# edwindn/rl-agent-for-qubit-array-tuning

Hardware: AMD Instinct MI355X
Metric: env steps/sec (batched 8-dot 64x64 CSD solves) (higher is better)
Workload: dtype f64; 1 GPU; 8-dot array, 4096 parallel envs per GPU, 64x64 CSD, deterministic physics (latching/noise off), 50-step episodes, staggered phases: 820 episode resets (new device + first observation) inside the timed region, synthetic CNN outputs; n_dots=8, envs_per_gpu=4096, resolution=64

## Files before the change

__graft_entry__.py:

```python
import os
import subprocess
import sys

ROOT = os.path.dirname(os.path.abspath(__file__))
PKG = os.path.join(ROOT, "rl-agent-for-qubit-array-tuning_amd")
for _p in (PKG, os.path.join(ROOT, "oracle"), os.path.join(ROOT, "tests")):
    if _p not in sys.path:
        sys.path.insert(0, _p)


def build() -> None:
    csrc = os.path.join(PKG, "csrc")
    subprocess.check_call(["make", "-C", csrc, "libqdsim.so"])
    subprocess.check_call(["make", "-C", os.path.join(ROOT, "tests", "hosttest"), "libqdsim_hosttest.so"])
    subprocess.check_call(["make", "-C", os.path.join(ROOT, "tests", "hosttest_wave"), "libqdsim_hosttest_wave.so"])
    subprocess.check_call(["make", "-C", os.path.join(ROOT, "oracle"), "libqdoracle.so"])
    import qadapt_hip
    from qadapt_hip import _lib
    L = _lib.lib()
    missing = [n for n in _lib.EXPORTS if not hasattr(L, n)]
    if missing:
        raise RuntimeError(f"libqdsim.so lacks symbols: {missing}")


def smoke() -> None:
    import numpy as np
    import torch
    import qd_oracle as O
    import helpers as H
    from qadapt_hip.vec_env import VecQuantumDeviceEnv, SyntheticCapacitanceModel

    assert torch.cuda.is_available(), "smoke() needs the MI355X"
    N, R, B, seed = 4, 16, 2, 2024
    env = VecQuantumDeviceEnv(B, num_dots=N, resolution=R, seed=seed, validate=True,
                              capacitance_model=SyntheticCapacitanceModel(3))
    rng = np.random.default_rng(0)
    C = N - 1
    v0 = rng.normal(0, 0.1, (B, C, 3)).astype(np.float32); l0 = rng.uniform(-6, -2, (B, C, 3)).astype(np.float32)
    obs = env.reset(cnn_outputs=(torch.as_tensor(v0).cuda(), torch.as_tensor(l0).cuda()))
    act = rng.uniform(-1, 1, (B, 2 * N - 1)).astype(np.float32)
    v1 = rng.normal(0, 0.1, (B, C, 3)).astype(np.float32); l1 = rng.uniform(-6, -2, (B, C, 3)).astype(np.float32)
    obs, rew, term, trunc = env.step(torch.as_tensor(act).cuda(),
                                     cnn_outputs=(torch.as_tensor(v1).cuda(), torch.as_tensor(l1).cuda()))
    img = obs["image"].cpu().numpy()
    raw, _ = env.raw()
    for e in range(B):
        oe = O.OracleEnv(N, R)
        oe.reset(O.sample_episode(np.random.default_rng(seed + e), N), v0[e], l0[e])
        oobs, (gr, br), _, _ = oe.step(act[e, :N], act[e, N:], v1[e], l1[e])
        r = rew[e].cpu().numpy()
        assert np.allclose(r[:N], gr, rtol=1e-9) and np.allclose(r[N:], br, rtol=1e-9), "reward mismatch"
        H.image_parity(oe, img[e], raw[e])
    env.close()
    print("smoke ok: 4-dot 16x16 batched step matches the oracle")


if __name__ == "__main__":
    build()
    if len(sys.argv) > 1 and sys.argv[1] == "smoke":
        smoke()
```

include/qdsim.h:

```cpp
#ifndef QDSIM_H
#define QDSIM_H

#include <stdint.h>

#ifdef __cplusplus
extern "C" {
#endif

#define QD_OK 0
#define QD_ERR_ARG 1
#define QD_ERR_HIP 2
#define QD_ERR_STATE 3
#define QD_ERR_NOMEM 4

#define QD_FLAG_VALIDATE 1
#define QD_FLAG_PIXEL_SEARCH 2
#define QD_FLAG_RETIRED_TILE_FUSED 4

#define QD_NOISE_SENSOR 1
#define QD_NOISE_RADIAL 2
#define QD_NOISE_LATCH 4

typedef struct qd_handle qd_handle;

typedef struct qd_config {
    int32_t struct_size;
    int32_t n_dot;
    int32_t resolution;
    int32_t batch;
    int32_t max_steps;
    int32_t env_chunk;
    int32_t flags;
    int32_t noise_flags;
    double gate_ramp_start;
    double gate_quadratic_start;
    double barrier_ramp_start;
    double kalman_prior_mean;
    double kalman_prior_variance;
    double kalman_prior_mean_nnn;
    double kalman_variance_threshold;
    double kalman_process_noise;
    uint64_t rng_seed;
    int64_t env_id_offset;
    int32_t use_deltas;
    int32_t sparse_reward;
    int32_t gate_curve_type;
    int32_t update_method;
    int32_t cnn_outputs;
    int32_t num_charge_states;
    double delta_max;
    double gate_curve_exponent;
    double plunger_radius;
    double outer_plunger_radius;
    double outer_plunger_reward_max;
    double barrier_radius;
} qd_config;

#define QD_ALL_CHARGE_STATES(m) (-(m))

#define QD_CURVE_CONSTANT 0
#define QD_CURVE_POLYNOMIAL 1
#define QD_CURVE_EXPONENTIAL 2
#define QD_CURVE_LINEAR 3
#define QD_UPDATE_KALMAN 0
#define QD_UPDATE_DIRECT 1

int qd_param_block_doubles(int n_dot);
int qd_state_block_doubles(int n_dot);
int qd_layout_query(int n_dot, int32_t* out31);
// ... 60 lines not shown
```

rl-agent-for-qubit-array-tuning_amd/csrc/qd_api.hip:

```cpp
#include <hip/hip_runtime.h>
#include <stdio.h>
#include <stdlib.h>
#include <string.h>
#include <new>

#include "qdsim.h"
#include "qd_kernels.h"
#include "qd_fullspace.h"
#include "qd_probe.h"

#define QD_MAX_LANES 4
struct QdLane {
    QdPixelRec* recs; unsigned char* slabs; unsigned* gtiles;
    unsigned char* wide;
    hipStream_t run, side, side2;
    hipEvent_t ev_fork, ev_join, ev_join2, ev_done;
};

struct qd_handle {
    qd_config cfg;
    QdLane lanes[QD_MAX_LANES]; int nlanes;
    hipEvent_t ev_start;
    int device;
    QdLayout L;
    int N, R, B, C, P;
    int chunk;
    double *params, *state, *zraw, *plohi, *occ, *eig;
    int* steps;
    QdPixelRec* recs;
    size_t recs_envs;
    float *gimg, *pimg, *bimg, *volt;
    unsigned long long* tel; int tel_words;
    unsigned long long* tstats;
    int tile_search;
    int kept, kc;
    int full_m;
    QdFullTab* ftab;
    int full_spl;
    QdWide wide;
    int ppb;
    unsigned char* slabs;
    unsigned* gtiles;
    int gs_chunk;
    size_t gs_batches;
    int cus;
    double* stage[2]; size_t stage_cap;
    hipEvent_t stage_ev[2]; int stage_turn;
    bool stage_busy[2];
    hipStream_t side, side2;
    hipEvent_t ev_fork, ev_join, ev_join2;
    unsigned long long obs_serial;
    double *pparams, *pstate, *pz, *pplohi;
    double *cz, *cplohi; size_t cz_cap, cplohi_cap;
    QdSelState* sel;
    char err[512];
};

static void qd_use_lane(qd_handle* h, int k) {
    const QdLane& ln = h->lanes[k];
    h->recs = ln.recs; h->slabs = ln.slabs; h->gtiles = ln.gtiles; h->wide.buf = ln.wide;
    h->side = ln.side; h->side2 = ln.side2; h->ev_fork = ln.ev_fork; h->ev_join = ln.ev_join; h->ev_join2 = ln.ev_join2;
}

static int qd_fail(qd_handle* h, int code, const char* what, hipError_t e = hipSuccess) {
    if (h) {
        if (e != hipSuccess) snprintf(h->err, sizeof(h->err), "%s: %s", what, hipGetErrorString(e));
        else snprintf(h->err, sizeof(h->err), "%s", what);
    }
    return code;
}
#define QD_HIP(call)                                                              \
    do { hipError_t e_ = (call); if (e_ != hipSuccess) return qd_fail(h, QD_ERR_HIP, #call, e_); } while (0)

struct QdDeviceGuard {
    int prev; bool switched; hipError_t err;
    explicit QdDeviceGuard(int dev) : prev(-1), switched(false), err(hipSuccess) {
        err = hipGetDevice(&prev);
        if (err == hipSuccess && prev != dev) { err = hipSetDevice(dev); switched = (err == hipSuccess); }
    }
    ~QdDeviceGuard() { if (switched) (void)hipSetDevice(prev); }
};
#define QD_ON_DEVICE(h)                                                           \
    QdDeviceGuard guard_((h)->device);                                            \
    if (guard_.err != hipSuccess) return qd_fail((h), QD_ERR_HIP, "hipSetDevice", guard_.err)

struct QdEventPair {
    hipEvent_t a, b; bool ok;
// ... 16 lines not shown
        case 8: { constexpr int NN = 8; __VA_ARGS__; } break;                            \
        default: return qd_fail(h, QD_ERR_ARG, "n_dot must be in 2..8");          \
    }

#define QD_DISPATCH_KC(KC_, ...)                                                  \
    switch (KC_) {                                                                \
        case 8: { constexpr int KK = 8; __VA_ARGS__; } break;                            \
        case 16: { constexpr int KK = 16; __VA_ARGS__; } break;                          \
        case 32: { constexpr int KK = 32; __VA_ARGS__; } break;                          \
        default: return qd_fail(h, QD_ERR_ARG, "kept-set size must be 8, 16 or 32");     \
    }

extern "C" int qd_param_block_doubles(int n) { return (n < 2 || n > QD_MAXN) ? -1 : qd_layout(n).size; }
extern "C" int qd_state_block_doubles(int n) { return (n < 2 || n > QD_MAXN) ? -1 : qd_layout(n).s_size; }
extern "C" int qd_layout_query(int n, int32_t* out) {
    if (n < 2 || n > QD_MAXN || !out) return QD_ERR_ARG;
    QdLayout L = qd_layout(n);
    memcpy(out, &L, sizeof(L));
    return QD_OK;
}

static void qd_kalman_priors(const qd_config& cfg, int N, double* km, double* kv) {
    for (int i = 0; i < N * N; ++i) { km[i] = 0.0; kv[i] = 0.0; }
    for (int i = 0; i < N - 1; ++i) {
        km[i * N + i + 1] = km[(i + 1) * N + i] = cfg.kalman_prior_mean;
        kv[i * N + i + 1] = kv[(i + 1) * N + i] = cfg.kalman_prior_variance;
    }
    if (cfg.cnn_outputs != 2)
        for (int i = 0; i < N - 2; ++i) {
            km[i * N + i + 2] = km[(i + 2) * N + i] = cfg.kalman_prior_mean_nnn;
            kv[i * N + i + 2] = kv[(i + 2) * N + i] = cfg.kalman_prior_variance;
        }
}

extern "C" const char* qd_last_error(const qd_handle* h) { return h ? h->err : "null handle"; }

extern "C" int qd_create(const qd_config* cfg, int device, qd_handle** out) {
    if (!cfg || !out || cfg->struct_size != (int32_t)sizeof(qd_config)) return QD_ERR_ARG;
    if (cfg->n_dot < 2 || cfg->n_dot > QD_MAXN || cfg->resolution < 2 || cfg->batch < 1) return QD_ERR_ARG;
    if (cfg->cnn_outputs != 2 && cfg->cnn_outputs != 3) return QD_ERR_ARG;
    if (cfg->gate_curve_type < 0 || cfg->gate_curve_type > 3 || cfg->update_method < 0 || cfg->update_method > 1) return QD_ERR_ARG;
    if (cfg->flags & QD_FLAG_RETIRED_TILE_FUSED) return QD_ERR_ARG;
    if (cfg->num_charge_states > QD_K) return QD_ERR_ARG;
    if (cfg->num_charge_states < 0 && !qd_full_supported(cfg->n_dot, -cfg->num_charge_states)) return QD_ERR_ARG;
    qd_handle* h = new (std::nothrow) qd_handle();
    if (!h) return QD_ERR_NOMEM;
    memset(h, 0, sizeof(*h));
    h->cfg = *cfg; h->device = device;
    h->N = cfg->n_dot; h->R = cfg->resolution; h->B = cfg->batch;
    h->C = h->N - 1; h->P = h->R * h->R; h->L = qd_layout(h->N);
    h->kept = cfg->num_charge_states > 0 ? cfg->num_charge_states : QD_K;
    h->kc = h->kept <= 8 ? 8 : (h->kept <= 16 ? 16 : 32);
    h->full_m = cfg->num_charge_states < 0 ? -cfg->num_charge_states : 0;
    *out = h;
    QD_ON_DEVICE(h);
    const bool val = (cfg->flags & QD_FLAG_VALIDATE) != 0;
    QdFullTab ftab;
    h->ppb = QD_GS_PPB;
    if (h->full_m) {
        qd_full_build(h->N, h->full_m, ftab);
        h->ppb = qd_full_ppb(ftab, val);
        if (h->ppb < 1) return qd_fail(h, QD_ERR_ARG, "the full charge-state space of this shape does not fit a slab");
        h->full_spl = qd_full_spl(ftab.M);
        if (qd_full_wide(ftab.maxsec)) h->wide.capw = (unsigned)((h->ppb * qd_full_wide_tasks(ftab) + 1) & ~1);
        QD_HIP(hipMalloc(&h->ftab, sizeof(QdFullTab)));
        QD_HIP(hipMemcpy(h->ftab, &ftab, sizeof(QdFullTab), hipMemcpyHostToDevice));
    }
    const size_t per_env_rec = (size_t)h->C * h->P * sizeof(QdPixelRec);
    const size_t batches_per_env = (size_t)h->C * ((h->P + h->ppb - 1) / h->ppb);
    const size_t per_env_slab = batches_per_env * (qd_gs_slab_bytes(val) + 4 * (qd_gs_tile_off(QD_GS_NBIN, 1)) + qd_wide_bytes(h->wide.capw));
    size_t budget = (size_t)64 << 30, free_b = 0, total_b = 0;
    if (const char* gib = getenv("QDSIM_SCRATCH_GIB")) { const long g = atol(gib); if (g > 0) budget = (size_t)g << 30; }
    if (hipMemGetInfo(&free_b, &total_b) == hipSuccess && free_b / 3 < budget) budget = free_b / 3;
    int chunk = cfg->env_chunk, gs_chunk;
    h->nlanes = 1;
    if (val) {
        chunk = h->B;
        size_t g = budget / per_env_slab;
        gs_chunk = (int)(g < 1 ? 1 : (g > (size_t)h->B ? (size_t)h->B : g));
        if (cfg->env_chunk > 0 && cfg->env_chunk < gs_chunk) gs_chunk = cfg->env_chunk;
    } else {
        h->nlanes = 2;
        if (const char* ls = getenv("QDSIM_LANES")) { const int l = atoi(ls); if (l >= 1 && l <= QD_MAX_LANES) h->nlanes = l; }
        if (chunk <= 0) {
            size_t g = budget / h->nlanes / (per_env_rec + per_env_slab);
            chunk = (int)(g < 1 ? 1 : g);
        }
        if (const char* cs = getenv("QDSIM_CHUNK")) { const int c = atoi(cs); if (c >= 1) chunk = c; }
        if (chunk >= h->B) {
            const int half = (h->B + 1) / 2;
            if (h->nlanes >= 2 && cfg->env_chunk <= 0 && (size_t)half * batches_per_env >= 2048) chunk = half;
            else { chunk = h->B; h->nlanes = 1; }
        }
        gs_chunk = chunk;
    }
    if ((size_t)gs_chunk * batches_per_env > ((size_t)1 << 20) - 1) {
        gs_chunk = (int)((((size_t)1 << 20) - 1) / batches_per_env);
        if (gs_chunk < 1) return qd_fail(h, QD_ERR_ARG, "resolution too large for the tile descriptors");
        if (!val && chunk > gs_chunk) chunk = gs_chunk;
    }
    h->chunk = chunk; h->recs_envs = (size_t)chunk;
    h->gs_chunk = gs_chunk; h->gs_batches = (size_t)gs_chunk * batches_per_env;
    {
        hipDeviceProp_t prop;
        QD_HIP(hipGetDeviceProperties(&prop, device));
        h->cus = prop.multiProcessorCount;
// ... 166 lines not shown
                   c.plunger_radius, c.outer_plunger_radius, c.outer_plunger_reward_max, c.barrier_radius};
    const int blk = 64, grd = (h->B + blk - 1) / blk;
    QD_DISPATCH_N(h->N, qd_k_actions<NN><<<dim3(grd), dim3(blk), 0, s>>>(h->B, h->params,
                                            h->state, h->steps, actions, rewards, truncated, rc));
    QD_HIP(hipGetLastError());
    return QD_OK;
}

static int qd_cand_blocks(int R) {
    const int tiles = ((R + 7) / 8) * ((R + 7) / 8), per_block = QD_CAND_BLOCK / 64;
    return (tiles + per_block - 1) / per_block;
}

static QdNoiseCfg qd_noise_cfg(const qd_handle* h) {
    QdNoiseCfg nz;
    nz.flags = h->cfg.noise_flags;
    nz.seed = (uint32_t)(h->cfg.rng_seed ^ (h->cfg.rng_seed >> 32));
    nz.env_off = (uint32_t)h->cfg.env_id_offset;
    nz.ser_lo = (uint32_t)h->obs_serial; nz.ser_hi = (uint32_t)(h->obs_serial >> 32);
    nz.tel = h->tel; nz.tel_words = h->tel_words;
    return nz;
}

template <int BIN>
static hipError_t qd_launch_solve(qd_handle* h, hipStream_t s) {
    static int per_cu[2] = {0, 0};
    const int v = h->eig ? 1 : 0;
    if (!per_cu[v]) {
        int n = 0;
        const hipError_t e = v ? hipOccupancyMaxActiveBlocksPerMultiprocessor(&n, qd_k_gs_solve<BIN, true>, 256, 0)
                               : hipOccupancyMaxActiveBlocksPerMultiprocessor(&n, qd_k_gs_solve<BIN, false>, 256, 0);
        if (e != hipSuccess) return e;
        per_cu[v] = n < 1 ? 1 : n;
    }
    const dim3 grid((unsigned)(h->cus * per_cu[v]));
    unsigned* tilelist = h->gtiles + 16;
    if (h->eig) qd_k_gs_solve<BIN, true><<<grid, dim3(256), 0, s>>>(h->slabs, h->gtiles, tilelist, h->gs_batches, h->tstats);
    else        qd_k_gs_solve<BIN, false><<<grid, dim3(256), 0, s>>>(h->slabs, h->gtiles, tilelist, h->gs_batches, nullptr);
    return hipGetLastError();
}

static int qd_launch_ground(qd_handle* h, const int32_t* env_ids, int base, int cnt, hipStream_t s, int stages = 7 ) {
    const int nb = (h->P + h->ppb - 1) / h->ppb;
    unsigned* tilelist = h->gtiles + 16;
    const int rec0 = (h->cfg.flags & QD_FLAG_VALIDATE) ? base : 0;
    for (int off = 0; off < cnt; off += h->gs_chunk) {
        const int n = cnt - off < h->gs_chunk ? cnt - off : h->gs_chunk;
        const QdGsGeom g{n, h->C, h->P, nb};
        const unsigned batches = (unsigned)((size_t)n * h->C * nb);
        if (stages & 1) {
        QD_HIP(hipMemsetAsync(h->gtiles, 0, sizeof(unsigned) * 16, s));
#define QD_LAUNCH_STRUCTURE(VAL_, WPB_)                                                                                          \
        QD_DISPATCH_N(h->N, qd_k_gs_structure<NN, VAL_, WPB_><<<dim3(batches), dim3(64 * WPB_), 0, s>>>(env_ids, base + off, rec0 + off, g, h->R, \
                      h->params, h->recs, h->state, h->cfg.noise_flags, h->slabs, h->gtiles, tilelist, h->gs_batches, h->kept))
        const bool small = batches < (unsigned)h->cus;
        if (h->full_m) {
#define QD_LAUNCH_FULL(VAL_, SPL_, WIDE_)                                                                                         \
            QD_DISPATCH_N(h->N, qd_k_full_structure<NN, VAL_, SPL_, WIDE_><<<dim3(batches), dim3(64 * QdFullWpb<SPL_>::v), 0, s>>>(env_ids,    \
                          base + off, rec0 + off, g, h->ppb, h->R, h->params, h->state, h->cfg.noise_flags, h->ftab, h->recs, h->slabs,   \
                          h->gtiles, tilelist, h->gs_batches, h->wide))
#define QD_LAUNCH_FULL_V(VAL_)                                                                                                    \
            do {                                                                                                                  \
                if (!h->wide.capw && h->full_spl == 2) { QD_LAUNCH_FULL(VAL_, 2, false); }                                        \
                else if (h->full_spl == 2) { QD_LAUNCH_FULL(VAL_, 2, true); }                                                     \
                else if (h->full_spl == 4) { QD_LAUNCH_FULL(VAL_, 4, true); }                                                     \
                else { QD_LAUNCH_FULL(VAL_, 8, true); }                                                                           \
            } while (0)
            if (h->eig) QD_LAUNCH_FULL_V(true); else QD_LAUNCH_FULL_V(false);
#undef QD_LAUNCH_FULL_V
#undef QD_LAUNCH_FULL
        } else if (h->eig) { if (small) { QD_LAUNCH_STRUCTURE(true, 16); } else { QD_LAUNCH_STRUCTURE(true, 4); } }
        else        { if (small) { QD_LAUNCH_STRUCTURE(false, 16); } else { QD_LAUNCH_STRUCTURE(false, 4); } }
#undef QD_LAUNCH_STRUCTURE
        QD_HIP(hipGetLastError());
        }
        if (stages & 2) {
        int max_bin = h->N == 2 ? qd_gs_bin(4) : (h->N == 3 ? qd_gs_bin(12) : QD_GS_NBIN - 1);
        if (h->full_m) {
            int M = 0, maxsec = 0;
            qd_full_sizes(h->N, h->full_m, M, maxsec);
            max_bin = qd_gs_bin(maxsec < QD_K ? maxsec : QD_K);
        } else if (h->kept < 2) max_bin = -1;
        else if (qd_gs_bin(h->kept) < max_bin) max_bin = qd_gs_bin(h->kept);
        const bool forked = max_bin >= 9;
        hipStream_t s9 = forked ? h->side : s, s48 = forked ? h->side2 : s;
        if (forked) {
            QD_HIP(hipEventRecord(h->ev_fork, s));
            QD_HIP(hipStreamWaitEvent(h->side, h->ev_fork, 0));
            QD_HIP(hipStreamWaitEvent(h->side2, h->ev_fork, 0));
        }
        if (h->wide.capw) {
            const size_t slots = (size_t)batches * h->wide.capw, full = (size_t)h->cus * 4;
            const dim3 wgrid((unsigned)(slots < full ? slots : full));
            if (h->eig) qd_k_full_solve_wide<true><<<wgrid, dim3(64), 0, s>>>(h->slabs, h->wide, batches, h->tstats);
            else        qd_k_full_solve_wide<false><<<wgrid, dim3(64), 0, s>>>(h->slabs, h->wide, batches, nullptr);
            QD_HIP(hipGetLastError());
        }
        if (max_bin >= 9) QD_HIP(qd_launch_solve<9>(h, s9));
        if (forked) QD_HIP(hipEventRecord(h->ev_join, h->side));
        if (max_bin >= 8) QD_HIP(qd_launch_solve<8>(h, s48));
        if (max_bin >= 7) QD_HIP(qd_launch_solve<7>(h, s48));
        if (max_bin >= 6) QD_HIP(qd_launch_solve<6>(h, s48));
        if (max_bin >= 5) QD_HIP(qd_launch_solve<5>(h, s48));
        if (max_bin >= 4) QD_HIP(qd_launch_solve<4>(h, s48));
        if (forked) QD_HIP(hipEventRecord(h->ev_join2, h->side2));
        if (max_bin >= 0) QD_HIP(qd_launch_solve<0>(h, s));
        if (max_bin >= 1) QD_HIP(qd_launch_solve<1>(h, s));
// ... 520 lines not shown
```

rl-agent-for-qubit-array-tuning_amd/csrc/qd_groundstate.h:

```cpp
#pragma once
#include "qd_pixel.h"
#include "qd_eig.h"

#if defined(__HIPCC__)

#ifndef QD_NBREG
#define QD_NBREG 6
#endif
#define QD_GS_BLOCK 256
#define QD_GS_PPB 256
#define QD_GS_NBIN 10
__host__ __device__ inline int qd_gs_bin(int s) { return s <= 8 ? s - 2 : (s <= 10 ? 7 : (s <= 12 ? 8 : 9)); }
__host__ __device__ inline int qd_gs_bin_min(int bin) { return bin <= 6 ? bin + 2 : (bin == 7 ? 9 : (bin == 8 ? 11 : 13)); }
#define QD_LINK_NONE 0xFFFFFFFFu
#define QD_LINK_SINGLE 0xFFFFFFFEu

typedef __attribute__((address_space(3))) double qd_lds_double;
typedef volatile qd_lds_double* qd_lds_vptr;
typedef const volatile qd_lds_double* qd_lds_cvptr;

template <int N>
struct QdWaveLds {
    static constexpr int NS = (2 * (N - 1) - QD_NBREG) > 1 ? (2 * (N - 1) - QD_NBREG) : 1;
    double coef[NS][64];
    unsigned char nidx[NS][64];
    double buf[64];
    double pv[2][16];
    short pfl[2][8];
};
struct QdBlockLds {
    unsigned pool_top;
    unsigned cnt[QD_GS_NBIN];
};

struct QdSlab {
    double* pool; unsigned* link; unsigned char* rank; unsigned* lists; double* aux; unsigned* cnt; double* lam;
};
__host__ __device__ inline int qd_gs_list_cap(int bin) { return QD_GS_PPB * (32 / qd_gs_bin_min(bin)); }
__host__ __device__ inline int qd_gs_list_off(int bin) { int o = 0; for (int b = 0; b < bin; ++b) o += qd_gs_list_cap(b); return o; }
__host__ __device__ inline int qd_gs_task_doubles(int s, bool validate) {
    const int ne = s * (s + 1) / 2;
    const int n = 2 + ne + (s > QD_EIG_REG ? 4 * s + (validate ? ne : 0) : 0);
    return (n + 1) & ~1;
}
__host__ __device__ inline size_t qd_gs_pool_doubles(bool validate) { return (size_t)QD_GS_PPB * (size_t)qd_gs_task_doubles(32, validate); }
__host__ __device__ inline size_t qd_gs_slab_bytes(bool validate) {
    size_t b = qd_gs_pool_doubles(validate) * 8;
    b += (size_t)QD_GS_PPB * 32 * 4;
    b += (size_t)qd_gs_list_off(QD_GS_NBIN) * 4;
    b += (size_t)QD_GS_PPB * 16;
    b += (size_t)QD_GS_PPB * 32;
    b += 64;
    b += (size_t)qd_gs_list_off(QD_GS_NBIN) * 8;
    return (b + 255) & ~(size_t)255;
}
__host__ __device__ inline QdSlab qd_gs_slab(unsigned char* base, bool validate) {
    QdSlab s;
    s.pool = (double*)base; base += qd_gs_pool_doubles(validate) * 8;
    s.link = (unsigned*)base; base += (size_t)QD_GS_PPB * 32 * 4;
    s.lists = (unsigned*)base; base += (size_t)qd_gs_list_off(QD_GS_NBIN) * 4;
    s.aux = (double*)base; base += (size_t)QD_GS_PPB * 16;
    s.rank = base; base += (size_t)QD_GS_PPB * 32;
    s.cnt = (unsigned*)base; base += 64;
    s.lam = (double*)base;
    return s;
}
__host__ __device__ inline size_t qd_gs_tile_cap(int bin, size_t batches) { return batches * (size_t)((qd_gs_list_cap(bin) + 63) / 64); }
__host__ __device__ inline size_t qd_gs_tile_off(int bin, size_t batches) { size_t o = 0; for (int b = 0; b < bin; ++b) o += qd_gs_tile_cap(b, batches); return o; }

__device__ __forceinline__ unsigned qd_half_ballot(bool p) {
    unsigned long long b = __ballot(p);
    return (unsigned)(b >> (threadIdx.x & 32));
}
__device__ __forceinline__ double qd_half_min(double v) {
#pragma unroll
    for (int o = 16; o > 0; o >>= 1) v = fmin(v, __shfl_xor(v, o, 32));
    return v;
}
__device__ __forceinline__ int qd_wave_max_int(int v) {
#pragma unroll
    for (int o = 32; o > 0; o >>= 1) v = max(v, __shfl_xor(v, o, 64));
    return __builtin_amdgcn_readfirstlane(v);
}

template <int N, bool VALIDATE>
__device__ __forceinline__ void qd_ground_structure(const QdPixelRec* __restrict__ rec, bool live, int ps, QdWaveLds<N>& W,
                                                    QdBlockLds& S, const QdSlab& sl, int kept) {
    const int lane = threadIdx.x & 63;
    const int m = lane & 31;
    const int hb = lane & 32;
    const unsigned lt = (1u << m) - 1u;
    qd_lds_vptr buf = (qd_lds_vptr)W.buf;

    const int hh = hb >> 5;
    if (m >= 9 && m < 9 + N - 1) W.pv[hh][m] = rec->tc[m - 9];
    if (m >= 16 && m < 16 + N) W.pfl[hh][m - 16] = (short)rec->fl[m - 16];
    __builtin_amdgcn_wave_barrier();
    const double* pvv = W.pv[hh];
    const bool inK = m < kept;
    const int nvalid = min(rec->nvalid, kept);
    const bool valid = m < nvalid;
    const unsigned code = valid ? (unsigned)rec->idx[m] : 0u;
    unsigned ecode = code;
    ecode = (ecode | (ecode << 8)) & 0x00FF00FFu;
    ecode = (ecode | (ecode << 4)) & 0x0F0F0F0Fu;
    ecode = (ecode | (ecode << 2)) & 0x33333333u;
    const double Fabs = inK ? rec->E[m] : INFINITY;
    const double fshift = qd_half_min(Fabs);
    const double F = Fabs - fshift;

    unsigned tcnz = 0;
#pragma unroll
    for (int d = 0; d < N - 1; ++d) tcnz |= (pvv[9 + d] != 0.0 ? 1u : 0u) << d;
    unsigned tcq = 0;
#pragma unroll
    for (int q = 0; q < N - 1; ++q) tcq |= ((tcnz >> (N - 2 - q)) & 1u) << (4 * q);
    unsigned nbrmask = 0;
#pragma unroll 4
    for (int j = 1; j <= 16; ++j) {
        const int pj = (m + j) & 31;
        const unsigned cj = __shfl(ecode, pj, 32);
        const unsigned Z = ((cj | 0x88888888u) - ecode) ^ 0x88888888u;
        const int tz = __builtin_ctz(Z | 0x80000000u);
        const unsigned Zs = Z >> tz;
        const unsigned hop = ((unsigned)(Zs == 0x1Fu) | (unsigned)(Zs == 0xF1u)) & (tcq >> tz) & 1u;
        nbrmask |= hop << pj;
        if (j < 16) {
            const int qj = (m - j) & 31;
            const unsigned back = (unsigned)__shfl((int)hop, qj, 32);
            nbrmask |= back << qj;
        }
    }
    nbrmask = (valid && live) ? (nbrmask & (nvalid >= 32 ? 0xFFFFFFFFu : ((1u << nvalid) - 1u))) : 0u;
#if defined(QD_ABLATE) && QD_ABLATE == 4
    nbrmask = 0;
#endif
    const int cnt = __popc(nbrmask);
    const int maxcnt = qd_wave_max_int(cnt);
    double radius = 0.0;
    double creg[QD_NBREG]; int jreg[QD_NBREG];
#pragma unroll
    for (int i = 0; i < QD_NBREG; ++i) { creg[i] = 0.0; jreg[i] = m; }
    {
        unsigned rem = nbrmask;
        for (int s = 0; s < maxcnt; ++s) {
            const bool has = rem != 0;
            const int j = has ? __builtin_ctz(rem) : m;
            rem &= rem - 1;
            const unsigned cj = __shfl(ecode, j, 32);
            double c = 0.0;
            if (has) {
                const int Y = (int)cj - (int)ecode;
                const unsigned ay = (unsigned)(Y < 0 ? -Y : Y);
                const int q = __builtin_ctz(ay) >> 2;
                const int d = N - 2 - q;
                const int nd = (int)W.pfl[hh][d] + (int)((ecode >> (4 * (q + 1))) & 3u) - 1;
                const int nd1 = (int)W.pfl[hh][d + 1] + (int)((ecode >> (4 * q)) & 3u) - 1;
                const double t = pvv[9 + d];
                const double prod = (Y < 0) ? (double)nd * ((double)nd1 + 1.0)
                                            : (double)nd1 * ((double)nd + 1.0);
                double sq_ = 0.0;
                if (prod > 0.0) sq_ = qd_sqrt1(prod);
                c = -t * sq_;
            }
            if (s < QD_NBREG) {
#pragma unroll
                for (int i = 0; i < QD_NBREG; ++i) if (i == s) { creg[i] = c; jreg[i] = j; }
            } else { W.coef[s - QD_NBREG][lane] = c; W.nidx[s - QD_NBREG][lane] = (unsigned char)j; }
            radius += fabs(c);
        }
    }

    unsigned seg = (1u << m) | nbrmask;
    for (int guard = 0; guard < 32; ++guard) {
        unsigned nw = seg, rem = nbrmask;
        for (int s = 0; s < maxcnt; ++s) {
            const bool has = rem != 0;
            const int j = has ? __builtin_ctz(rem) : m;
            rem &= rem - 1;
            nw |= __shfl(seg, j, 32);
        }
        const bool changed = nw != seg;
        seg = nw;
        if (!__any(changed)) break;
    }
    const int ssz = __popc(seg);
    const int r = __popc(seg & lt);
    const int smax = qd_wave_max_int(ssz);

    double comp_lower;
    {
        buf[lane] = F - radius;
        __builtin_amdgcn_wave_barrier();
        double acc = INFINITY;
        unsigned mm = seg;
        for (int it = 0; it < smax; ++it) {
            if (mm) { const int b = __builtin_ctz(mm); mm &= mm - 1; acc = fmin(acc, buf[hb + b]); }
        }
        __builtin_amdgcn_wave_barrier();
        comp_lower = acc;
    }
    const bool active = live && comp_lower <= 0.0;
#if defined(QD_ABLATE) && QD_ABLATE == 3
    const bool solve = false;
#else
    const bool solve = active && ssz > 1;
#endif

    unsigned base = 0, gi = 0;
    if (solve && r == 0) {
        base = atomicAdd(&S.pool_top, (unsigned)qd_gs_task_doubles(ssz, VALIDATE));
        const int bin = qd_gs_bin(ssz);
        gi = (unsigned)qd_gs_list_off(bin) + atomicAdd(&S.cnt[bin], 1u);
        sl.lists[gi] = base;
        if (ssz > 8) sl.pool[base + 1] = (double)ssz;
    }
    base = (unsigned)__shfl((int)base, __builtin_ctz(seg), 32);
    gi = (unsigned)__shfl((int)gi, __builtin_ctz(seg), 32);
    if (live) {
        sl.link[ps * 32 + m] = solve ? gi : (active ? QD_LINK_SINGLE : QD_LINK_NONE);
        sl.rank[ps * 32 + m] = (unsigned char)r;
        if (VALIDATE) {
            const double hn = -qd_half_min(inK ? -(fabs(Fabs) + radius) : INFINITY);
            if (m == 0) { sl.aux[ps] = hn; sl.aux[QD_GS_PPB + ps] = fshift; }
        }
    }
    {
        double* row = sl.pool + base + 2 + (r * (r + 1)) / 2;
        unsigned nrm = 0;
        for (int s = 0; s < maxcnt; ++s) {
            if (s < cnt && solve) {
                int j = jreg[0]; double c = creg[0];
                if (s >= QD_NBREG) { j = (int)W.nidx[s - QD_NBREG][lane]; c = W.coef[s - QD_NBREG][lane]; }
#pragma unroll
                for (int i = 1; i < QD_NBREG; ++i) if (i == s) { j = jreg[i]; c = creg[i]; }
                const int rj = __popc(seg & ((1u << j) - 1u));
                if (rj < r) { row[rj] = c; nrm |= 1u << rj; }
            }
        }
        for (int c = 0; c < smax - 1; ++c)
            if (solve && c < r && !((nrm >> c) & 1u)) row[c] = 0.0;
        if (solve) row[r] = F;
    }
}

template <int S, bool PADDED, bool VALIDATE>
__device__ __forceinline__ int qd_eig_task(double* rec, double& lam) {
    double resid, x[S];
    int its = 0;
    const int sz = PADDED ? (int)rec[1] : S;
    qd_eig_lowest<S, VALIDATE>(rec + 2, lam, x, resid, VALIDATE ? &its : nullptr, sz);
    if (VALIDATE) rec[1] = resid;
    if (sz == S) {
        double2* X2 = reinterpret_cast<double2*>(rec + 2);
#pragma unroll
// ... 102 lines not shown
```

rl-agent-for-qubit-array-tuning_amd/csrc/qd_kernels.h:

```cpp
#pragma once
#include "qd_groundstate.h"
#include "qd_rng.h"

#if defined(__HIPCC__)

struct QdRewardCfg {
    double gate_ramp_start, gate_quadratic_start, barrier_ramp_start;
    int max_steps;
    int use_deltas, sparse, curve;
    double delta_max, curve_exponent;
    double plunger_radius, outer_plunger_radius, outer_plunger_reward_max, barrier_radius;
};

__device__ __forceinline__ double qd_gate_reward(double dist, const QdRewardCfg& rc) {
    if (rc.sparse) {
        if (dist <= rc.plunger_radius) return 1.0;
        if (dist <= rc.outer_plunger_radius) {
            const double nd = (dist - rc.plunger_radius) / (rc.outer_plunger_radius - rc.plunger_radius);
            return rc.outer_plunger_reward_max * (1.0 - nd);
        }
        return 0.0;
    }
    double r;
    if (dist >= rc.gate_ramp_start) r = 0.0;
// ... 163 lines not shown
    if (nv < KC) {
        double dd[N];
#pragma unroll
        for (int i = 0; i < N; ++i) dd[i] = 0.0 - vd[i];
#pragma unroll 1
        for (int i = 0; i < N; ++i) {
            const double t = qd_dotN<N>(spar + L.cdd_inv + i * G, dd);
            double di = dd[0];
#pragma unroll
            for (int j = 1; j < N; ++j) di = (j == i) ? dd[j] : di;
            F0 = fma(di, t, F0);
        }
    }
#pragma unroll
    for (int m = 0; m < KC; ++m) rec->E[m] = (m < nv ? se[m * QD_CAND_BLOCK + threadIdx.x] : F0) * isa;
#pragma unroll
    for (int i = 0; i < N; ++i) rec->fl[i] = fl[i];
    rec->nvalid = nv;
}

struct QdGsGeom { int n_env, C, P, nb; };
__device__ __forceinline__ void qd_gs_locate(const QdGsGeom& g, int batch, int& slot, int& ch, int& p0) {
    slot = batch / (g.C * g.nb);
    const int rem = batch - slot * g.C * g.nb;
    ch = rem / g.nb; p0 = (rem - ch * g.nb) * QD_GS_PPB;
}

__device__ __forceinline__ void qd_gs_publish_tiles(const QdBlockLds& sB, const QdSlab& sl, int batch, unsigned* __restrict__ gtiles,
                                                    unsigned* __restrict__ tilelist, size_t batches_cap) {
    if (threadIdx.x < QD_GS_NBIN) {
        const int bin = threadIdx.x;
        const unsigned nt = sB.cnt[bin];
        sl.cnt[bin] = nt;
        const unsigned ntile = (nt + 63u) >> 6;
        if (ntile) {
            const unsigned start = atomicAdd(&gtiles[bin], ntile);
            unsigned* tl = tilelist + qd_gs_tile_off(bin, batches_cap) + start;
            for (unsigned t = 0; t < ntile; ++t) {
                const unsigned here = nt - t * 64u < 64u ? nt - t * 64u : 64u;
                tl[t] = ((unsigned)batch << 12) | (t << 6) | (here - 1u);
            }
        }
    }
}

#ifndef QD_GS_WAVES
#define QD_GS_WAVES 7
#endif
template <int N, bool VALIDATE, int WPB>
__global__ void __launch_bounds__(64 * WPB, WPB == 4 ? QD_GS_WAVES : 4)
qd_k_gs_structure(const int* __restrict__ env_ids, int env_base, int rec_slot0, QdGsGeom g, int R, const double* __restrict__ params,
                  const QdPixelRec* __restrict__ recs, const double* __restrict__ state, int noise_flags,
                  unsigned char* __restrict__ slabs, unsigned* __restrict__ gtiles, unsigned* __restrict__ tilelist, size_t batches_cap,
                  int kept) {
    const QdLayout L = qd_layout(N);
    __shared__ QdWaveLds<N> sW[WPB];
    __shared__ QdBlockLds sB;
    constexpr int PPW = QD_GS_PPB / WPB;
    const int batch = blockIdx.x;
    const QdSlab sl = qd_gs_slab(slabs + (size_t)batch * qd_gs_slab_bytes(VALIDATE), VALIDATE);
    const int wave = threadIdx.x >> 6, lane = threadIdx.x & 63;
    int slot, ch, p0;
    qd_gs_locate(g, batch, slot, ch, p0);
    const int e = env_ids ? env_ids[env_base + slot] : env_base + slot;
    const double* par = params + (size_t)e * L.size;
    const double* st = state + (size_t)e * L.s_size;
    if (qd_radial_replaced(par, st, L, ch, noise_flags)) {
        if (threadIdx.x < QD_GS_NBIN) sl.cnt[threadIdx.x] = 0;
        return;
    }
    const QdPixelRec* rbase = recs + ((size_t)(rec_slot0 + slot) * g.C + ch) * g.P;
    if (threadIdx.x <= QD_GS_NBIN) { if (threadIdx.x == 0) sB.pool_top = 0; else sB.cnt[threadIdx.x - 1] = 0; }
    __syncthreads();
    QdWaveLds<N>& W = sW[wave];
    for (int it = 0; it < PPW / 2; ++it) {
        const int ps = wave * PPW + it * 2 + (lane >> 5);
        if (p0 + wave * PPW + it * 2 >= g.P) break;
        const int p = p0 + ps;
        const int pc = p < g.P ? p : g.P - 1;
        qd_ground_structure<N, VALIDATE>(rbase + pc, p < g.P, ps, W, sB, sl, kept);
    }
    __syncthreads();
    qd_gs_publish_tiles(sB, sl, batch, gtiles, tilelist, batches_cap);
}

template <int BIN, bool VALIDATE>
__device__ __forceinline__ int qd_gs_solve_task(double* rec, double& lam) {
    if constexpr (BIN <= 6) return qd_eig_task<BIN + 2, false, VALIDATE>(rec, lam);
    else if constexpr (BIN == 7) return qd_eig_task<10, true, VALIDATE>(rec, lam);
    else if constexpr (BIN == 8) return qd_eig_task<12, true, VALIDATE>(rec, lam);
    else return qd_eig_task_mem<VALIDATE>(rec, lam);
}
template <int BIN> struct QdGsSolveWaves { static constexpr int v = BIN <= 1 ? 6 : (BIN == 2 ? 4 : (BIN == 3 ? 3 : (BIN <= 6 ? 2 : (BIN == 9 ? 4 : 1)))); };

template <int BIN, bool VALIDATE>
__global__ void __launch_bounds__(256, QdGsSolveWaves<BIN>::v)
qd_k_gs_solve(unsigned char* __restrict__ slabs, const unsigned* __restrict__ gtiles, const unsigned* __restrict__ tilelist,
              size_t batches_cap, unsigned long long* __restrict__ stats) {
    const int lane = threadIdx.x & 63;
    const unsigned ntile = gtiles[BIN];
    const unsigned* tl = tilelist + qd_gs_tile_off(BIN, batches_cap);
    const unsigned nwaves = gridDim.x * 4u;
    unsigned gt = blockIdx.x * 4u + (threadIdx.x >> 6);
    const size_t slab_bytes = qd_gs_slab_bytes(VALIDATE);
    auto offset_of = [&](unsigned d) -> unsigned {
        const QdSlab sl = qd_gs_slab(slabs + (size_t)(d >> 12) * slab_bytes, VALIDATE);
        return lane <= (int)(d & 63u) ? sl.lists[qd_gs_list_off(BIN) + (int)((d >> 6) & 63u) * 64 + lane] : 0u;
    };
    unsigned desc = gt < ntile ? tl[gt] : 0u;
    unsigned desc1 = gt + nwaves < ntile ? tl[gt + nwaves] : 0u;
    unsigned off = gt < ntile ? offset_of(desc) : 0u;
    for (; gt < ntile; gt += nwaves) {
        const unsigned desc2 = gt + 2u * nwaves < ntile ? tl[gt + 2u * nwaves] : 0u;
        const unsigned off1 = gt + nwaves < ntile ? offset_of(desc1) : 0u;
        const unsigned batch = desc >> 12;
        const int here = (int)(desc & 63u) + 1;
        const QdSlab sl = qd_gs_slab(slabs + (size_t)batch * slab_bytes, VALIDATE);
        int its = 0;
        if (lane < here) {
            double lam;
            its = qd_gs_solve_task<BIN, VALIDATE>(sl.pool + off, lam);
            sl.lam[qd_gs_list_off(BIN) + (int)((desc >> 6) & 63u) * 64 + lane] = lam;
        }
        desc = desc1; desc1 = desc2; off = off1;
        if (VALIDATE && stats) {
            int sum = its, mx = its;
#pragma unroll
            for (int o = 32; o > 0; o >>= 1) { sum += __shfl_xor(sum, o, 64); mx = max(mx, __shfl_xor(mx, o, 64)); }
            if (lane == 0) {
                atomicAdd(&stats[16], (unsigned long long)here); atomicAdd(&stats[17], (unsigned long long)sum);
                atomicAdd(&stats[18], 1ull); atomicAdd(&stats[19], (unsigned long long)mx);
                atomicAdd(&stats[20 + BIN], (unsigned long long)here);
            }
// ... 579 lines not shown
```

rl-agent-for-qubit-array-tuning_amd/qadapt_hip/_lib.py:

```python
from __future__ import annotations

import ctypes
import os
import subprocess

_HERE = os.path.dirname(os.path.abspath(__file__))
CSRC = os.path.join(os.path.dirname(_HERE), "csrc")
LIB_PATH = os.environ.get("QDSIM_LIB", os.path.join(CSRC, "libqdsim.so"))

QD_FLAG_VALIDATE = 1
QD_FLAG_PIXEL_SEARCH = 2
QD_NOISE_SENSOR = 1
QD_NOISE_RADIAL = 2
QD_NOISE_LATCH = 4
QD_MAP_GLOBAL, QD_MAP_PER_SCAN = 0, 1
QD_ERR_ARG, QD_ERR_HIP, QD_ERR_STATE = 1, 2, 3

EXPORTS = [
    "qd_param_block_doubles", "qd_state_block_doubles", "qd_layout_query", "qd_create", "qd_destroy",
    "qd_last_error", "qd_bind_outputs", "qd_load_episodes", "qd_apply_actions", "qd_observe",
    "qd_update_capacitance", "qd_step", "qd_snapshot", "qd_get_state", "qd_set_state", "qd_get_raw",
    "qd_get_occupations", "qd_get_candidates", "qd_get_eigen", "qd_get_search_stats", "qd_get_solver_stats", "qd_get_rng_state", "qd_set_rng_state",
    "qd_time_ground_kernel", "qd_time_candidates_kernel", "qd_time_kernels", "qd_timed_kernel_name", "qd_chunk_envs",
    "qd_probe", "qd_probe_compose", "qd_time_select",
]

QD_CURVES = {"constant": 0, "polynomial": 1, "exponential": 2, "linear": 3}
QD_UPDATE_KALMAN, QD_UPDATE_DIRECT = 0, 1


class QdConfig(ctypes.Structure):
    _fields_ = [
        ("struct_size", ctypes.c_int32), ("n_dot", ctypes.c_int32), ("resolution", ctypes.c_int32),
        ("batch", ctypes.c_int32), ("max_steps", ctypes.c_int32), ("env_chunk", ctypes.c_int32),
        ("flags", ctypes.c_int32), ("noise_flags", ctypes.c_int32),
        ("gate_ramp_start", ctypes.c_double), ("gate_quadratic_start", ctypes.c_double),
        ("barrier_ramp_start", ctypes.c_double), ("kalman_prior_mean", ctypes.c_double),
        ("kalman_prior_variance", ctypes.c_double), ("kalman_prior_mean_nnn", ctypes.c_double),
        ("kalman_variance_threshold", ctypes.c_double), ("kalman_process_noise", ctypes.c_double),
        ("rng_seed", ctypes.c_uint64), ("env_id_offset", ctypes.c_int64),
        ("use_deltas", ctypes.c_int32), ("sparse_reward", ctypes.c_int32), ("gate_curve_type", ctypes.c_int32),
        ("update_method", ctypes.c_int32), ("cnn_outputs", ctypes.c_int32), ("num_charge_states", ctypes.c_int32),
        ("delta_max", ctypes.c_double), ("gate_curve_exponent", ctypes.c_double),
        ("plunger_radius", ctypes.c_double), ("outer_plunger_radius", ctypes.c_double),
        ("outer_plunger_reward_max", ctypes.c_double), ("barrier_radius", ctypes.c_double),
    ]


class QdError(RuntimeError):
    pass


def build(force=False):
    if force and os.path.exists(LIB_PATH):
        os.remove(LIB_PATH)
    subprocess.check_call(["make", "-s", "-C", CSRC, "libqdsim.so"])
    return LIB_PATH


_LIB = None


def lib():
    global _LIB
# ... 59 lines not shown
```

rl-agent-for-qubit-array-tuning_amd/qadapt_hip/vec_env.py:

```python
from __future__ import annotations

import ctypes

import numpy as np
import torch

from . import _lib
from .device_model import DeviceSampler, check_solver_options, load_yaml, max_charge_carriers
from .layout import layout


class SyntheticCapacitanceModel:

    def __init__(self, seed=99, outputs=3):
        self.seed = seed
        self.calls = 0
        self.outputs = outputs

    def __call__(self, images):
        n = images.shape[0]
        g = torch.Generator(device="cpu").manual_seed(self.seed + self.calls)
        self.calls += 1
        values = torch.randn((n, self.outputs), generator=g, dtype=torch.float32) * 0.1
        log_vars = torch.rand((n, self.outputs), generator=g, dtype=torch.float32) * 4.0 - 6.0
# ... 9 lines not shown
            "current_barrier_voltages": st[:, L.s_barrier_v:L.s_barrier_v + N - 1].copy(),
            "virtual_gate_matrix": st[:, L.s_vgm:L.s_vgm + G * G].reshape(-1, G, G).copy(),
            "virtual_gate_origin": params[:, L.origin:L.origin + G].copy(),
            "kalman_means": st[:, L.s_kmean:L.s_kmean + N * N].reshape(-1, N, N).copy(),
            "kalman_variances": st[:, L.s_kvar:L.s_kvar + N * N].reshape(-1, N, N).copy(),
            "steps": steps}


def cgd_full_from_params(L, params):
    return params[:, L.cgd:L.cgd + L.G * L.V].reshape(-1, L.G, L.V).copy()


def override_charge_states(qconfig, num_charge_states):
    if num_charge_states is not None:
        qconfig["simulator"].setdefault("latched_model", {})["num_charge_states"] = \
            None if num_charge_states == "all" else num_charge_states
    return qconfig


def make_qd_config(config, qconfig, num_dots, resolution, batch, *, env_chunk=0, flags=0, noise_flags=0, seed=0,
                   env_id_offset=0):
    sim, rew, cm = config["simulator"], config["reward"], config["capacitance_model"]
    nearest = bool(cm.get("nearest_neighbour"))
    k = check_solver_options(qconfig, n_dot=num_dots)
    ncs = k if k is not None else -max_charge_carriers(qconfig)
    return _lib.QdConfig(struct_size=ctypes.sizeof(_lib.QdConfig), n_dot=int(num_dots), resolution=int(resolution),
                         batch=int(batch), max_steps=int(sim["max_steps"]), env_chunk=int(env_chunk), flags=int(flags),
                         noise_flags=int(noise_flags),
                         gate_ramp_start=float(rew["gate_ramp_start"]),
                         gate_quadratic_start=float(rew["gate_quadratic_start"]),
                         barrier_ramp_start=float(rew["barrier_ramp_start"]),
                         kalman_prior_mean=0.3, kalman_prior_variance=0.5, kalman_prior_mean_nnn=0.15,
                         kalman_variance_threshold=float(cm.get("variance_threshold", 0.05)),
                         kalman_process_noise=float(cm.get("process_noise", 0.0)),
                         rng_seed=int(seed) & 0xFFFFFFFFFFFFFFFF, env_id_offset=int(env_id_offset),
                         use_deltas=1 if sim.get("use_deltas") else 0,
                         sparse_reward=1 if rew.get("sparse_reward") else 0,
                         gate_curve_type=_lib.QD_CURVES[rew.get("gate_curve_type", "constant")],
                         update_method=_lib.QD_UPDATE_DIRECT if cm["update_method"] == "direct" else _lib.QD_UPDATE_KALMAN,
                         cnn_outputs=2 if nearest else 3, num_charge_states=ncs,
                         delta_max=float(sim.get("delta_max", 0.0)),
                         gate_curve_exponent=float(rew.get("gate_curve_exponent", 2.0)),
                         plunger_radius=float(rew.get("plunger_radius", 0.0)),
                         outer_plunger_radius=float(rew.get("outer_plunger_radius", 0.0)),
                         outer_plunger_reward_max=float(rew.get("outer_plunger_reward_max", 0.0)),
                         barrier_radius=float(rew.get("barrier_radius", 0.0)))


class VecQuantumDeviceEnv:
    def __init__(self, num_envs, num_dots=None, config_path=None, qarray_config_path=None,
                 resolution=None, device=None, seed=None, env_id_offset=0, capacitance_model=None,
                 validate=False, env_chunk=0, reset_kalman_on_reset=False, noise=None,
                 vary_peak_width=False, peak_width_alpha=0.01, voltage_capacitance_model=None, pixel_search=False,
                 num_charge_states=None):
        if seed is None:
            seed = int(np.random.SeedSequence().entropy) & 0x7FFFFFFFFFFF
        self.seed = int(seed)
        self.env_id_offset = int(env_id_offset)
        self.config = load_yaml(config_path, "env_config.yaml")
        self.qconfig = load_yaml(qarray_config_path, "qarray_config.yaml")
        override_charge_states(self.qconfig, num_charge_states)
        if voltage_capacitance_model is not None:
            self.qconfig["simulator"]["voltage_capacitance_model"]["type"] = \
                None if voltage_capacitance_model in ("none", "null") else voltage_capacitance_model
        sim = self.config["simulator"]
        self.num_envs = int(num_envs)
        self.num_dots = int(num_dots if num_dots is not None else sim["num_dots"])
        self.num_charge_states = check_solver_options(self.qconfig, n_dot=self.num_dots)
        self.max_charge_carriers = max_charge_carriers(self.qconfig) if self.num_charge_states is None else None
        self.use_barriers = bool(sim["use_barriers"])
        if not self.use_barriers:
            raise NotImplementedError("env.py only supports barrier mode for now")
        rew = self.config["reward"]
        if rew.get("gate_curve_type", "constant") not in _lib.QD_CURVES:
            raise ValueError(f"Unknown curve type: {rew.get('gate_curve_type')}")
        self.resolution = int(resolution if resolution is not None else sim["resolution"])
        self.max_steps = int(sim["max_steps"])
        self.update_method = self.config["capacitance_model"]["update_method"]
        if self.update_method in ("bayesian", "kriging", "ema"):
            raise NotImplementedError(f"update_method={self.update_method!r} requires an updater module the "
                                      "reference removed; use 'kalman' or 'direct'")
        if self.update_method == "fake":
            raise ValueError("update_method 'fake' fails in the reference's barrier mode (shape mismatch in "
                             "QarrayBaseClass._update_virtual_gate_matrix); not built")
        if self.update_method not in (None, "kalman", "direct", "perfect"):
            raise ValueError(f"Unknown update method: {self.update_method}")
        self.nearest_neighbour = bool(self.config["capacitance_model"].get("nearest_neighbour"))
        self.cnn_outputs = 2 if self.nearest_neighbour else 3
        if self.update_method in (None, "perfect"):
            capacitance_model = None
        self.capacitance_model = capacitance_model
        if self.update_method in ("kalman", "direct") and capacitance_model is None:
            raise RuntimeError("Error initialising capacitance model: update_method 'kalman' needs a "
                               "capacitance_model callable (images -> values, log_vars)")
        if not torch.cuda.is_available():
            raise RuntimeError("VecQuantumDeviceEnv needs a ROCm GPU (no CPU fallback)")
        self.device = torch.device(device if device is not None else "cuda")
        if self.device.index is None:
            self.device = torch.device("cuda", torch.cuda.current_device())
        self.reset_kalman_on_reset = bool(reset_kalman_on_reset)
        N = self.num_dots; R = self.resolution; B = self.num_envs
        self.N, self.R, self.B, self.C = N, R, B, N - 1
        self.L = layout(N)
        self.sampler = DeviceSampler(N, self.qconfig, self.config, vary_peak_width=vary_peak_width,
                                     peak_width_alpha=peak_width_alpha,
                                     perfect_vgm=self.update_method == "perfect")
        self._rngs = [np.random.Generator(np.random.PCG64(self.seed + self.env_id_offset + e)) for e in range(B)]
        self._lib = _lib.lib()
        cfg = make_qd_config(self.config, self.qconfig, N, R, B, env_chunk=env_chunk,
                             flags=(_lib.QD_FLAG_VALIDATE if validate else 0) | (_lib.QD_FLAG_PIXEL_SEARCH if pixel_search else 0),
                             noise_flags=self._noise_flags(noise), seed=self.seed, env_id_offset=self.env_id_offset)
        self._h = ctypes.c_void_p()
        rc = self._lib.qd_create(ctypes.byref(cfg), self.device.index, ctypes.byref(self._h))
        if rc != 0:
            msg = self._lib.qd_last_error(self._h).decode() if self._h else "no handle"
            if self._h:
                self._lib.qd_destroy(self._h)
                self._h = None
            raise _lib.QdError(f"qd_create failed (code {rc}): {msg}")
        self.validate = bool(validate)
        dev = self.device
        self.global_image = torch.zeros((B, R, R, self.C), dtype=torch.float32, device=dev)
        self.plunger_images = torch.zeros((B, N, R, R, 2), dtype=torch.float32, device=dev)
        self.barrier_images = torch.zeros((B, self.C, R, R, 1), dtype=torch.float32, device=dev)
        self.voltages = torch.zeros((B, 2 * N - 1), dtype=torch.float32, device=dev)
        self.rewards = torch.zeros((B, 2 * N - 1), dtype=torch.float64, device=dev)
        self.truncated = torch.zeros((B,), dtype=torch.uint8, device=dev)
        _lib.check(self._h, self._lib.qd_bind_outputs(self._h, self.global_image.data_ptr(),
                                                      self.plunger_images.data_ptr(),
                                                      self.barrier_images.data_ptr(),
                                                      self.voltages.data_ptr()), "qd_bind_outputs")
        self._params_host = np.zeros((B, self.L.size))
        self._steps_host = np.zeros(B, np.int64)
        self._needs_reset = True
        self.obs_count = 0
        self.final = None

    def _noise_flags(self, noise):
        if not noise:
            return 0
        if noise is True:
            rn = self.config["simulator"].get("radial_noise") or {}
            lt = self.qconfig["simulator"]["model"].get("latching_model_parameters") or {}
            return (_lib.QD_NOISE_SENSOR | (_lib.QD_NOISE_RADIAL if rn.get("enabled") else 0)
                    | (_lib.QD_NOISE_LATCH if lt.get("Exists") else 0))
        f = 0
        for k in noise:
            f |= {"sensor": _lib.QD_NOISE_SENSOR, "radial": _lib.QD_NOISE_RADIAL, "latch": _lib.QD_NOISE_LATCH}[k]
        return f

    def _stream(self):
        return ctypes.c_void_p(torch.cuda.current_stream(self.device).cuda_stream)

    def close(self):
        if getattr(self, "_h", None) is not None and self._h:
            self._lib.qd_destroy(self._h)
            self._h = None

    def __del__(self):
        try:
            self.close()
        except Exception:
            pass
# ... 284 lines not shown
```

Baseline: 12310 env-steps/s.

## Prune ground-state components using pairwise 2x2 eigenvalue upper bound

In the ground-state structure pass, each lane now tracks the best neighbour pair and computes an upper bound on the minimum energy from the 2x2 pair eigenvalue. Components whose Gershgorin lower bound exceeds this bound (plus a small scale-relative margin) are marked inactive, and singleton components with positive diagonal are skipped. This is meant to cut the number of per-pixel components that reach the expensive eigen-solve. The cost is extra per-lane arithmetic, an LDS write and shuffles, and a risk to correctness if the margin is too tight. An optional min-F mode, set by a flag or environment variable, uses the threshold 0 instead.

```diff
diff --git a/__graft_entry__.py b/__graft_entry__.py
--- a/__graft_entry__.py
+++ b/__graft_entry__.py
@@ -14,6 +14,7 @@
     subprocess.check_call(["make", "-C", csrc, "libqdsim.so"])
     subprocess.check_call(["make", "-C", os.path.join(ROOT, "tests", "hosttest"), "libqdsim_hosttest.so"])
     subprocess.check_call(["make", "-C", os.path.join(ROOT, "tests", "hosttest_wave"), "libqdsim_hosttest_wave.so"])
+    subprocess.check_call(["make", "-C", os.path.join(ROOT, "tests", "hosttest_prune"), "libqdsim_hosttest_prune.so"])
     subprocess.check_call(["make", "-C", os.path.join(ROOT, "oracle"), "libqdoracle.so"])
     import qadapt_hip
     from qadapt_hip import _lib
diff --git a/include/qdsim.h b/include/qdsim.h
--- a/include/qdsim.h
+++ b/include/qdsim.h
@@ -15,6 +15,7 @@
 
 #define QD_FLAG_VALIDATE 1
 #define QD_FLAG_PIXEL_SEARCH 2
+#define QD_FLAG_PRUNE_MINF 8
 #define QD_FLAG_RETIRED_TILE_FUSED 4
 
 #define QD_NOISE_SENSOR 1
diff --git a/rl-agent-for-qubit-array-tuning_amd/csrc/qd_api.hip b/rl-agent-for-qubit-array-tuning_amd/csrc/qd_api.hip
--- a/rl-agent-for-qubit-array-tuning_amd/csrc/qd_api.hip
+++ b/rl-agent-for-qubit-array-tuning_amd/csrc/qd_api.hip
@@ -33,6 +33,7 @@
     unsigned long long* tel; int tel_words;
     unsigned long long* tstats;
     int tile_search;
+    int gsflags;
     int kept, kc;
     int full_m;
     QdFullTab* ftab;
@@ -155,6 +156,8 @@
     h->kept = cfg->num_charge_states > 0 ? cfg->num_charge_states : QD_K;
     h->kc = h->kept <= 8 ? 8 : (h->kept <= 16 ? 16 : 32);
     h->full_m = cfg->num_charge_states < 0 ? -cfg->num_charge_states : 0;
+    h->gsflags = (cfg->flags & QD_FLAG_PRUNE_MINF) ? QD_GS_PRUNE_MINF : 0;
+    if (const char* pr = getenv("QDSIM_PRUNE")) { if (!strcmp(pr, "minf")) h->gsflags |= QD_GS_PRUNE_MINF; }
     *out = h;
     QD_ON_DEVICE(h);
     const bool val = (cfg->flags & QD_FLAG_VALIDATE) != 0;
@@ -427,7 +430,7 @@
         QD_HIP(hipMemsetAsync(h->gtiles, 0, sizeof(unsigned) * 16, s));
 #define QD_LAUNCH_STRUCTURE(VAL_, WPB_)                                                                                          \
         QD_DISPATCH_N(h->N, qd_k_gs_structure<NN, VAL_, WPB_><<<dim3(batches), dim3(64 * WPB_), 0, s>>>(env_ids, base + off, rec0 + off, g, h->R, \
-                      h->params, h->recs, h->state, h->cfg.noise_flags, h->slabs, h->gtiles, tilelist, h->gs_batches, h->kept))
+                      h->params, h->recs, h->state, h->cfg.noise_flags, h->slabs, h->gtiles, tilelist, h->gs_batches, h->kept, h->gsflags))
         const bool small = batches < (unsigned)h->cus;
         if (h->full_m) {
 #define QD_LAUNCH_FULL(VAL_, SPL_, WIDE_)                                                                                         \
diff --git a/rl-agent-for-qubit-array-tuning_amd/csrc/qd_groundstate.h b/rl-agent-for-qubit-array-tuning_amd/csrc/qd_groundstate.h
--- a/rl-agent-for-qubit-array-tuning_amd/csrc/qd_groundstate.h
+++ b/rl-agent-for-qubit-array-tuning_amd/csrc/qd_groundstate.h
@@ -1,6 +1,7 @@
 #pragma once
 #include "qd_pixel.h"
 #include "qd_eig.h"
+#include "qd_prune.h"
 
 #if defined(__HIPCC__)
 
@@ -14,6 +15,10 @@
 __host__ __device__ inline int qd_gs_bin_min(int bin) { return bin <= 6 ? bin + 2 : (bin == 7 ? 9 : (bin == 8 ? 11 : 13)); }
 #define QD_LINK_NONE 0xFFFFFFFFu
 #define QD_LINK_SINGLE 0xFFFFFFFEu
+#define QD_GS_PRUNE_MINF 1
+#ifndef QD_PRUNE_SQRT
+#define QD_PRUNE_SQRT 1
+#endif
 
 typedef __attribute__((address_space(3))) double qd_lds_double;
 typedef volatile qd_lds_double* qd_lds_vptr;
@@ -85,7 +90,7 @@
 
 template <int N, bool VALIDATE>
 __device__ __forceinline__ void qd_ground_structure(const QdPixelRec* __restrict__ rec, bool live, int ps, QdWaveLds<N>& W,
-                                                    QdBlockLds& S, const QdSlab& sl, int kept) {
+                                                    QdBlockLds& S, const QdSlab& sl, int kept, int gsflags) {
     const int lane = threadIdx.x & 63;
     const int m = lane & 31;
     const int hb = lane & 32;
@@ -138,6 +143,9 @@
     const int cnt = __popc(nbrmask);
     const int maxcnt = qd_wave_max_int(cnt);
     double radius = 0.0;
+    buf[lane] = F;
+    __builtin_amdgcn_wave_barrier();
+    double pbest = INFINITY, pF = F, pc = 0.0;
     double creg[QD_NBREG]; int jreg[QD_NBREG];
 #pragma unroll
     for (int i = 0; i < QD_NBREG; ++i) { creg[i] = 0.0; jreg[i] = m; }
@@ -162,6 +170,9 @@
                 double sq_ = 0.0;
                 if (prod > 0.0) sq_ = qd_sqrt1(prod);
                 c = -t * sq_;
+                const double Fj = buf[hb + j];
+                const double p2 = qd_prune_pair_proxy2(F, Fj, c);
+                if (p2 < pbest) { pbest = p2; pF = Fj; pc = c; }
             }
             if (s < QD_NBREG) {
 #pragma unroll
@@ -170,6 +181,15 @@
             radius += fabs(c);
         }
     }
+    double Ul = INFINITY;
+    if (cnt) Ul = QD_PRUNE_SQRT ? qd_prune_pair_bound(F, pF, pc) : 0.5 * pbest;
+    const double U = fmin(0.0, qd_half_min(Ul));
+    const bool minf = (gsflags & QD_GS_PRUNE_MINF) != 0;
+    const bool anchor = !minf && U < 0.0 && Ul == U;
+    int hhi = qd_prune_hi(inK ? F + radius : 0.0);
+#pragma unroll
+    for (int o = 16; o > 0; o >>= 1) hhi = max(hhi, __shfl_xor(hhi, o, 32));
+    const double U_safe = minf ? 0.0 : qd_prune_threshold(U, qd_prune_scale(hhi));
 
     unsigned seg = (1u << m) | nbrmask;
     for (int guard = 0; guard < 32; ++guard) {
@@ -190,7 +210,8 @@
 
     double comp_lower;
     {
-        buf[lane] = F - radius;
+        __builtin_amdgcn_wave_barrier();
+        buf[lane] = anchor ? -INFINITY : F - radius;
         __builtin_amdgcn_wave_barrier();
         double acc = INFINITY;
         unsigned mm = seg;
@@ -200,7 +221,7 @@
         __builtin_amdgcn_wave_barrier();
         comp_lower = acc;
     }
-    const bool active = live && comp_lower <= 0.0;
+    const bool active = live && !(comp_lower > U_safe) && (ssz > 1 || F <= 0.0);
 #if defined(QD_ABLATE) && QD_ABLATE == 3
     const bool solve = false;
 #else
diff --git a/rl-agent-for-qubit-array-tuning_amd/csrc/qd_kernels.h b/rl-agent-for-qubit-array-tuning_amd/csrc/qd_kernels.h
--- a/rl-agent-for-qubit-array-tuning_amd/csrc/qd_kernels.h
+++ b/rl-agent-for-qubit-array-tuning_amd/csrc/qd_kernels.h
@@ -239,7 +239,7 @@
 qd_k_gs_structure(const int* __restrict__ env_ids, int env_base, int rec_slot0, QdGsGeom g, int R, const double* __restrict__ params,
                   const QdPixelRec* __restrict__ recs, const double* __restrict__ state, int noise_flags,
                   unsigned char* __restrict__ slabs, unsigned* __restrict__ gtiles, unsigned* __restrict__ tilelist, size_t batches_cap,
-                  int kept) {
+                  int kept, int gsflags) {
     const QdLayout L = qd_layout(N);
     __shared__ QdWaveLds<N> sW[WPB];
     __shared__ QdBlockLds sB;
@@ -265,7 +265,7 @@
         if (p0 + wave * PPW + it * 2 >= g.P) break;
         const int p = p0 + ps;
         const int pc = p < g.P ? p : g.P - 1;
-        qd_ground_structure<N, VALIDATE>(rbase + pc, p < g.P, ps, W, sB, sl, kept);
+        qd_ground_structure<N, VALIDATE>(rbase + pc, p < g.P, ps, W, sB, sl, kept, gsflags);
     }
     __syncthreads();
     qd_gs_publish_tiles(sB, sl, batch, gtiles, tilelist, batches_cap);
diff --git a/rl-agent-for-qubit-array-tuning_amd/csrc/qd_prune.h b/rl-agent-for-qubit-array-tuning_amd/csrc/qd_prune.h
--- /dev/null
+++ b/rl-agent-for-qubit-array-tuning_amd/csrc/qd_prune.h
@@ -0,0 +1,24 @@
+#pragma once
+#include "qd_eig.h"
+
+#define QD_PRUNE_MARGIN 4e-12
+
+QD_HD double qd_prune_pair_proxy2(double Fi, double Fj, double c) {
+    return (Fi + Fj) - fmax(2.0 * fabs(c), fabs(Fi - Fj));
+}
+QD_HD double qd_prune_pair_bound(double Fi, double Fj, double c) {
+    const double a = 0.5 * (Fi + Fj), d = 0.5 * (Fi - Fj);
+    const double ss = d * d + c * c;
+    double root = fmax(fabs(c), fabs(d));
+    if (ss > 1e-280 && ss < 1e280) root = qd_sqrt1(ss);
+    return a - root;
+}
+QD_HD int qd_prune_hi(double v) {
+    union { double d; unsigned long long u; } c; c.d = v;
+    return (int)(c.u >> 32);
+}
+QD_HD double qd_prune_scale(int hi) {
+    union { double d; unsigned long long u; } c; c.u = (unsigned long long)(unsigned)(hi + 1) << 32;
+    return c.d;
+}
+QD_HD double qd_prune_threshold(double U, double scale) { return U + QD_PRUNE_MARGIN * scale; }
diff --git a/rl-agent-for-qubit-array-tuning_amd/qadapt_hip/_lib.py b/rl-agent-for-qubit-array-tuning_amd/qadapt_hip/_lib.py
--- a/rl-agent-for-qubit-array-tuning_amd/qadapt_hip/_lib.py
+++ b/rl-agent-for-qubit-array-tuning_amd/qadapt_hip/_lib.py
@@ -10,6 +10,7 @@
 
 QD_FLAG_VALIDATE = 1
 QD_FLAG_PIXEL_SEARCH = 2
+QD_FLAG_PRUNE_MINF = 8
 QD_NOISE_SENSOR = 1
 QD_NOISE_RADIAL = 2
 QD_NOISE_LATCH = 4
diff --git a/rl-agent-for-qubit-array-tuning_amd/qadapt_hip/vec_env.py b/rl-agent-for-qubit-array-tuning_amd/qadapt_hip/vec_env.py
--- a/rl-agent-for-qubit-array-tuning_amd/qadapt_hip/vec_env.py
+++ b/rl-agent-for-qubit-array-tuning_amd/qadapt_hip/vec_env.py
@@ -85,7 +85,7 @@
                  resolution=None, device=None, seed=None, env_id_offset=0, capacitance_model=None,
                  validate=False, env_chunk=0, reset_kalman_on_reset=False, noise=None,
                  vary_peak_width=False, peak_width_alpha=0.01, voltage_capacitance_model=None, pixel_search=False,
-                 num_charge_states=None):
+                 num_charge_states=None, prune_min_f=False):
         if seed is None:
             seed = int(np.random.SeedSequence().entropy) & 0x7FFFFFFFFFFF
         self.seed = int(seed)
@@ -141,7 +141,8 @@
         self._rngs = [np.random.Generator(np.random.PCG64(self.seed + self.env_id_offset + e)) for e in range(B)]
         self._lib = _lib.lib()
         cfg = make_qd_config(self.config, self.qconfig, N, R, B, env_chunk=env_chunk,
-                             flags=(_lib.QD_FLAG_VALIDATE if validate else 0) | (_lib.QD_FLAG_PIXEL_SEARCH if pixel_search else 0),
+                             flags=(_lib.QD_FLAG_VALIDATE if validate else 0) | (_lib.QD_FLAG_PIXEL_SEARCH if pixel_search else 0)
+                             | (_lib.QD_FLAG_PRUNE_MINF if prune_min_f else 0),
                              noise_flags=self._noise_flags(noise), seed=self.seed, env_id_offset=self.env_id_offset)
         self._h = ctypes.c_void_p()
         rc = self._lib.qd_create(ctypes.byref(cfg), self.device.index, ctypes.byref(self._h))
```

Result: slower. 12010 env-steps/s (-2.5%).
